# michaelwillett/GPU-ICP-SLAM

Hardware: AMD Instinct MI355X
Metric: particle-scan evals/sec (1081 beams x N particles), full particleFilter step, KD path (higher is better)
Workload: dtype f32; 1 GPU; synthetic 1081-beam scans, 100000 particles/GPU, 100000-point KD map, full SLAM step (disperse+score+weights+ICP/SVD+map update+resample); particles_global=100000, parallelism=particles sharded x1, map replicated, kd_size_end=191383

## Files before the change

gpu-icp-slam_amd/csrc/kd_cells.hip.inc:

```

#define PF_CELL_SUB 2
#define PF_CELL_WIN (2560 * PF_CELL_SUB)
#define PF_CELL_LIST_CAP (1 << 19)
#define PF_CELL_POOL_CAP (1 << 22)
#define PF_CELL_MAXC 12
#define PF_CELL_RUN 32
#define PF_CELL_MAXR 14
#define PF_CELL_MARK_MAX 4096
#define PF_CELL_PENDING 0xFFFFFFFFu
#define PF_CELL_FALLBACK 0xFFFFFFFEu
enum { PF_CS_COUNT = 0, PF_CS_POOL, PF_CS_SNAP, PF_CS_PAD3, PF_CS_LIST_CAP, PF_CS_POOL_CAP, PF_CS_FLAGS, PF_CS_PAD, PF_CS_ROWS, PF_CS_N1, PF_CS_N2,
       PF_CS_NONE, PF_CS_CUR_FRESH, PF_CS_CUR_EXT, PF_CS_CUR_REUSED, PF_CS_CUR_CLAIMED, PF_CS_WORDS = 32,
       PF_CS_OX = 128, PF_CS_OY = 129, PF_CS_ALLOC = 256 };
#define PF_CF_LIST_FULL 1
#define PF_CF_POOL_FULL 2
#define PF_CF_NEED_ORIGIN 4
#define PF_CF_FAR 8
#define PF_CELL_DRIFT_MAX 120
#define PF_REC_WORDS 96
#define PF_REC_TERM 4
#define PF_REC_CAND 20
#define PF_REC_PAR 36
#define PF_REC_RC 52
#define PF_REC_POOL 76
// ... 40 lines not shown
    const int k = S >> 1;
    cell_lo = (float)k * res;
    const float mid = cell_lo + 0.5f * res;
    lo = (S & 1) ? mid : cell_lo;
    hi = (S & 1) ? (float)(k + 1) * res : mid;
}
static_assert(PF_CELL_SUB == 2, "sub_index / sub_edges halve the lattice cell");

__device__ __forceinline__ bool beam_box(const pf::KdGroupBox &b, int j, float r, float &wxlo, float &wxhi, float &wylo, float &wyhi,
                                         const pf::AngleParts *T = nullptr, const pf::BeamParts *beams = nullptr)
{
    const float tc = 0.5f * (b.tlo + b.thi), dth = 0.5f * (b.thi - b.tlo);
    float cx, cy;
    if (T) beam_end_point(beams, j, r, tc, *T, cx, cy);
    else pf::clean_lidar_scan(j, r, tc, cx, cy);
    const float dd = dth + 1e-6f;
    const float eps = 2e-4f + 1e-5f * fabsf(r) + fabsf(r) * 2.0f * 1.1920929e-7f * (fabsf(tc) + 2.4f + dd);
    const float hx = (fabsf(cy) + fabsf(r) * dd) * dd + eps, hy = (fabsf(cx) + fabsf(r) * dd) * dd + eps;
    wxlo = b.xlo + cx - hx; wxhi = b.xhi + cx + hx; wylo = b.ylo + cy - hy; wyhi = b.yhi + cy + hy;
    return (wxlo == wxlo) && (wxhi == wxhi) && (wylo == wylo) && (wyhi == wyhi) && fabsf(wxlo) < 1e6f && fabsf(wxhi) < 1e6f &&
           fabsf(wylo) < 1e6f && fabsf(wyhi) < 1e6f && (wxhi - wxlo) < 4.0f && (wyhi - wylo) < 4.0f && fabsf(r) < PF_RANGE_NEVER;
}

#define PF_MARK_THREADS 256
#define PF_MARK_GROUPS 8
#define PF_MARK_CLAIMS 2048
#define PF_MARK_WORDS 4096
__global__ __launch_bounds__(PF_MARK_THREADS) void k_cells_mark(const pf::KdGroupBox *__restrict__ box, int groups,
                                                                const float *__restrict__ scan, int nb, CellGeom geo, unsigned *tab,
                                                                int *__restrict__ list, int *cs, const pf::AngleParts *__restrict__ gparts,
                                                                const pf::BeamParts *__restrict__ beams, unsigned long long *__restrict__ probe = nullptr)
{
    pf_stamp(probe);
    __shared__ unsigned bm[PF_MARK_WORDS];
    __shared__ int s_red[4][PF_MARK_THREADS / 64];
    const int t = threadIdx.x, lane = t & 63, wave = t >> 6, j = blockIdx.x;
    const int ox = cs[PF_CS_OX], oy = cs[PF_CS_OY];
    const float r = scan[j];
    int kx0[PF_MARK_GROUPS], kx1[PF_MARK_GROUPS], ky0[PF_MARK_GROUPS], ky1[PF_MARK_GROUPS];
    int ux0 = INT_MAX, ux1 = INT_MIN, uy0 = INT_MAX, uy1 = INT_MIN;
#pragma unroll
    for (int q = 0; q < PF_MARK_GROUPS; q++) {
        const int g = blockIdx.y * (PF_MARK_THREADS * PF_MARK_GROUPS) + q * PF_MARK_THREADS + t;
        kx0[q] = ky0[q] = INT_MAX;
        kx1[q] = ky1[q] = INT_MIN;
        if (g < groups) {
            float wxlo, wxhi, wylo, wyhi;
            const pf::AngleParts T = gparts[g];
            if (beam_box(box[g], j, r, wxlo, wxhi, wylo, wyhi, &T, beams)) {
                const int okx = ox >> 1, oky = oy >> 1, wk = PF_CELL_WIN / PF_CELL_SUB;
                const int a0 = max(lattice_floor(wxlo, geo.resx, geo.invx) - okx, 0), a1 = min(lattice_floor(wxhi, geo.resx, geo.invx) - okx, wk - 1);
                const int b0 = max(lattice_floor(wylo, geo.resy, geo.invy) - oky, 0), b1 = min(lattice_floor(wyhi, geo.resy, geo.invy) - oky, wk - 1);
                if (a0 <= a1 && b0 <= b1 && (long long)(a1 - a0 + 1) * (b1 - b0 + 1) <= PF_CELL_MARK_MAX) {
                    kx0[q] = a0; kx1[q] = a1; ky0[q] = b0; ky1[q] = b1;
// ... 4 lines not shown
    }
    for (int off = 32; off >= 1; off >>= 1) {
        ux0 = min(ux0, __shfl_xor(ux0, off, 64)); ux1 = max(ux1, __shfl_xor(ux1, off, 64));
        uy0 = min(uy0, __shfl_xor(uy0, off, 64)); uy1 = max(uy1, __shfl_xor(uy1, off, 64));
    }
    if (lane == 0) { s_red[0][wave] = ux0; s_red[1][wave] = ux1; s_red[2][wave] = uy0; s_red[3][wave] = uy1; }
    __syncthreads();
    for (int k = 0; k < PF_MARK_THREADS / 64; k++) {
        ux0 = min(ux0, s_red[0][k]); ux1 = max(ux1, s_red[1][k]); uy0 = min(uy0, s_red[2][k]); uy1 = max(uy1, s_red[3][k]);
    }
    if (ux0 > ux1) return;
    const int nx = ux1 - ux0 + 1;
    const long long bits = (long long)nx * (uy1 - uy0 + 1);
    __shared__ int s_claim[PF_MARK_CLAIMS];
    __shared__ int s_nclaim, s_base;
    if (t == 0) s_nclaim = 0;
    __syncthreads();
    auto claim = [&](int idx) {
        if (atomicCAS(&tab[idx], 0u, PF_CELL_PENDING) == 0u) {
            const int k = atomicAdd(&s_nclaim, 1);
            if (k < PF_MARK_CLAIMS) s_claim[k] = idx;
            else {
                const int pos = atomicAdd(&cs[PF_CS_COUNT], 1);
                if (pos < cs[PF_CS_LIST_CAP]) list[pos] = idx;
                else {
                    atomicExch(&tab[idx], PF_CELL_FALLBACK);
                    atomicOr(&cs[PF_CS_FLAGS], PF_CF_LIST_FULL);
                }
            }
        }
    };
    auto flush = [&]() {
        __syncthreads();
        const int nc = min(s_nclaim, PF_MARK_CLAIMS);
        if (t == 0 && nc > 0) {
            s_base = atomicAdd(&cs[PF_CS_COUNT], nc);
            atomicAdd(&cs[PF_CS_CUR_CLAIMED], nc);
        }
        __syncthreads();
        for (int k = t; k < nc; k += PF_MARK_THREADS) {
            const int pos = s_base + k;
            if (pos < cs[PF_CS_LIST_CAP]) list[pos] = s_claim[k];
            else {
                atomicExch(&tab[s_claim[k]], PF_CELL_FALLBACK);
                atomicOr(&cs[PF_CS_FLAGS], PF_CF_LIST_FULL);
            }
        }
    };
    if (bits > (long long)PF_MARK_WORDS * 32) {
#pragma unroll
        for (int q = 0; q < PF_MARK_GROUPS; q++) {
            if (kx0[q] > kx1[q] || (long long)(kx1[q] - kx0[q] + 1) * (ky1[q] - ky0[q] + 1) > PF_CELL_MARK_MAX) continue;
            for (int cy = ky0[q]; cy <= ky1[q]; cy++)
                for (int cx = kx0[q]; cx <= kx1[q]; cx++) claim(2 * cy * PF_CELL_WIN + 2 * cx);
        }
        flush();
        return;
    }
    const int words = (int)((bits + 31) >> 5);
    for (int w = t; w < words; w += PF_MARK_THREADS) bm[w] = 0u;
    __syncthreads();
#pragma unroll
    for (int q = 0; q < PF_MARK_GROUPS; q++)
        for (int cy = ky0[q]; cy <= ky1[q]; cy++) {
            const int b0 = (cy - uy0) * nx - ux0 + kx0[q], b1 = b0 + (kx1[q] - kx0[q]);
            for (int w = b0 >> 5; w <= (b1 >> 5); w++) {
// ... 624 lines not shown
#undef S_RY
__device__ __forceinline__ float cell_dist2(const uint4 cd, float wx, float wy)
{
    typedef float f32x2 __attribute__((ext_vector_type(2)));
    const f32x2 nxy = {__uint_as_float(cd.x), __uint_as_float(cd.y)};
    const f32x2 pxy = {wx, wy};
    const f32x2 d = nxy - pxy;
    const f32x2 dd = d * d;
    return dd.x + dd.y;
}
__device__ __forceinline__ bool cell_visit(const uint4 cd, float wx, float wy, float &sBest)
{
    const float s = cell_dist2(cd, wx, wy);
    const float sGuard = sBest * PF_GUARD_K;
    bool take = s < sGuard;
    const bool inBand = (s < sBest) != take;
    if (__builtin_amdgcn_ballot_w64(inBand) != 0ull) {
        float sb = sBest;
        asm volatile("" : "+v"(sb));
        take = take | (inBand && pf::fsqrt(s) < pf::fsqrt(sb));
    }
    sBest = take ? s : sBest;
    return take;
}

#define PF_ROW_SLACK 4
template <bool CENSUS = false, int GUARD = 1>
__global__ __launch_bounds__(64) void k_score_kd_cells(const float *__restrict__ px, const float *__restrict__ py,
                                                       const float *__restrict__ pth, int n, const float *__restrict__ scan,
                                                       const pf::BeamParts *__restrict__ beams, int nb, int beams_per_chunk, pf::KdView tree,
                                                       CellGeom geo, const unsigned *__restrict__ tab, const uint4 *__restrict__ pool,
                                                       const int *__restrict__ cs, const int *__restrict__ order, int direct,
                                                       float *__restrict__ out, int out_mode, pf::KdCensus *__restrict__ census = nullptr,
                                                       unsigned long long *__restrict__ probe = nullptr, const double2 *__restrict__ tparts = nullptr)
{
    pf_stamp(probe);
    const int g = blockIdx.x, slot = g * 64 + threadIdx.x;
    const int j0 = blockIdx.y * beams_per_chunk;
    const int j1 = min(nb, j0 + beams_per_chunk);
    const bool real = slot < n;
    const int i = order ? order[min(slot, n - 1)] : min(slot, n - 1);
    const float x = px[i], y = py[i], th = pth[i];
    pf::AngleParts T;
    if (tparts) {
        const double2 tp = tparts[i];
        T.c = tp.x;
// ... 144 lines not shown
```

gpu-icp-slam_amd/csrc/pfslam_frame.hip.inc:

```

#define PF_FRAME_RING 4
enum { PF_FS_BOUND = 0, PF_FS_WALKED = 4, PF_FS_TICKET = 8, PF_FS_ICP = 9, PF_FS_WORDS = 16 };
enum { PF_WC_WALLS = 0, PF_WC_NEW, PF_WC_FLAGS, PF_WC_SIZE, PF_WC_WORDS = 4 };

enum { PF_FL_REDUCED = 0, PF_FL_TREE, PF_FL_ORDER, PF_FL_ICP, PF_FL_SCAN, PF_FL_FTAIL, PF_FL_POSEG , PF_FL_WORDS = 8 };
__device__ __forceinline__ void flag_store(int *word, int ticket) { __hip_atomic_store(word, ticket, __ATOMIC_RELEASE, __HIP_MEMORY_SCOPE_AGENT); }
__device__ __forceinline__ bool flag_wait(const int *word, int ticket, int *err)
{
    const unsigned long long t0 = wall_clock64(), limit = g_gate_ticks;
    while (__hip_atomic_load(word, __ATOMIC_ACQUIRE, __HIP_MEMORY_SCOPE_AGENT) - ticket < 0) {
        __builtin_amdgcn_s_sleep(8);
        if (wall_clock64() - t0 > limit) {
            if (err) __hip_atomic_store(err, ticket, __ATOMIC_RELAXED, __HIP_MEMORY_SCOPE_SYSTEM);
            return false;
        }
    }
    return true;
}
__global__ void k_gate(const int *__restrict__ word, int ticket, int *__restrict__ err)
{
    if (threadIdx.x == 0) flag_wait(word, ticket, err);
}
__global__ void k_gate_signal(int *__restrict__ done_word, int done_ticket, const int *__restrict__ word, int ticket, int *__restrict__ err)
{
    if (threadIdx.x != 0) return;
    flag_store(done_word, done_ticket);
// ... 421 lines not shown
            wy = roundf(pf::fdiv(wy, resy));
            wx += (float)cx;
            wy += (float)cy;
            if (wx >= 0 && wx < dimx && wy >= 0 && wy < dimy) key = (uint32_t)(int)(wx * dimx + wy);
        }
    }
#pragma unroll
    for (int k = 2; k <= 64; k <<= 1)
#pragma unroll
        for (int q = k >> 1; q > 0; q >>= 1) {
            const uint32_t other = (uint32_t)__shfl_xor((int)key, q, 64);
            const bool asc = (lane & k) == 0, lower = (lane & q) == 0;
            key = (lower == asc) ? min(key, other) : max(key, other);
        }
    runs_g[j] = key;
    keys_s[j] = 0xFFFFFFFFu;
    if (probe && blockIdx.x == 0 && lane == 0) probe[PB_WALLS_KEYS - PB_WALLS] = wall_clock64();
}

template <bool PLANAR>
__global__ __launch_bounds__(64) void k_walls_rank_traverse(const uint32_t *__restrict__ runs_g, int sort_n, const float *__restrict__ pose, int dimx, float resx,
                                                            float resy, float scalex, float scaley, pf::KdView tree, uint32_t *__restrict__ keys_s,
                                                            float2 *__restrict__ xy_s, int *__restrict__ c2_s, int *__restrict__ leaf_s,
                                                            int *__restrict__ new_s, unsigned long long *__restrict__ probe, int split)
{
    pf_stamp(probe);
    extern __shared__ uint32_t s_dyn[];
    uint32_t *runs = s_dyn;
    const int lane = threadIdx.x, n_runs = sort_n >> 6, mine = blockIdx.x / split, per = 64 / split, pos = (blockIdx.x % split) * per + lane;
    for (int i = lane; i < sort_n; i += 64) runs[i] = runs_g[i];
    __syncthreads();
    if (lane >= per) return;
    const int i = mine * 64 + pos;
    const uint32_t key = runs[i];
    if (key == 0xFFFFFFFFu) return;
    int rank = pos;
    bool dup = pos > 0 && runs[i - 1] == key;
    for (int r0 = 0; r0 < n_runs; r0 += 4) {
        int lo[4] = {0, 0, 0, 0};
        uint32_t pk[4];
        bool on[4];
#pragma unroll
        for (int u = 0; u < 4; u++) {
            const int r = r0 + u;
            on[u] = r < n_runs && r != mine && !(r > mine && key == 0u);
            pk[u] = r < mine ? key : key - 1u;
        }
#pragma unroll
        for (int step = 32; step >= 1; step >>= 1)
#pragma unroll
            for (int u = 0; u < 4; u++)
                if (on[u]) lo[u] += (runs[(r0 + u) * 64 + lo[u] + step - 1] <= pk[u]) ? step : 0;
#pragma unroll
        for (int u = 0; u < 4; u++)
            if (on[u]) {
                const int cnt = lo[u] + ((lo[u] == 63 && runs[(r0 + u) * 64 + 63] <= pk[u]) ? 1 : 0);
                rank += cnt;
                if (r0 + u < mine && cnt > 0 && runs[(r0 + u) * 64 + cnt - 1] == key) dup = true;
            }
    }
    if (dup) return;
    const float4 p = cell_to_point((int)key, dimx, resx, resy, scalex, scaley, pose[0], pose[1]);
    int leaf;
    const int b = pf::kd_resume<PLANAR, false, true>(tree, p.x, p.y, p.z, INFINITY, 0, 0, nullptr, &leaf);
    const float cellDiag = pf::fsqrt(resx * resx + resy * resy), minDist = cellDiag / 2.0f;
    keys_s[rank] = key;
    xy_s[rank] = make_float2(p.x, p.y);
    c2_s[rank] = b;
    leaf_s[rank] = leaf;
    new_s[rank] = node_dist(tree, b, p) > minDist ? 1 : 0;
}

template <bool PLANAR>
__global__ __launch_bounds__(256) void k_free_traverse(float4 *__restrict__ free_pts, int *__restrict__ free_idx, int free_cap, int wall_cap,
                                                       const int *__restrict__ counts, pf::KdView tree, int zero_tail, float *kw, float resx,
                                                       float resy, const int *__restrict__ bound_ptr, unsigned long long *__restrict__ probe)
{
    pf_stamp(probe);
    const int n_wall = min(counts[0], wall_cap), n_free = min(counts[1], free_cap);
    const int bound = *bound_ptr;
    const float cellDiag = pf::fsqrt(resx * resx + resy * resy);
    for (int i = blockIdx.x * 256 + threadIdx.x; i < n_free; i += gridDim.x * 256) {
        float4 p = free_pts[i];
        if (zero_tail && i >= n_wall) {
            p = make_float4(0.0f, 0.0f, 0.0f, 0.0f);
            free_pts[i] = p;
        }
// ... 517 lines not shown
                     c.multi ? (const long long *)h->gkeys : (const long long *)nullptr, c.multi ? (const float *)h->gpose : (const float *)nullptr, h->world, h->stride};
    return c;
}
#define FV_EDGE_WAIT(st, word, ev, back)                                                                                                      \
    do {                                                                                                                                      \
        if (c.gates) {                                                                                                                        \
            hipLaunchKernelGGL(k_gate, dim3(1), dim3(64), 0, st, (const int *)(c.fl + (word)), seq - (back), h->gate_err_dev);                \
            HIPCHK(hipGetLastError());                                                                                                        \
        } else HIPCHK(hipStreamWaitEvent(st, ev, 0));                                                                                         \
    } while (0)

static int fv_cells_passes(pfslam_handle *h, const FvCtx &c)
{
    const int seq = c.seq, s4 = c.s4, groups = c.groups;
    hipStream_t K = c.K;
    const bool mark_early = h->mark_early != 0;
    if (!c.sync_cells) {
        if (mark_early) FV_EDGE_WAIT(K, PF_FL_ORDER, h->ev_order, 0);
        else FV_EDGE_WAIT(K, PF_FL_REDUCED, h->ev_reduced, 0);
    }
    hipLaunchKernelGGL(k_group_box, dim3(groups), dim3(64), 0, K, h->x_frame, h->y_frame, h->th_frame, h->n, (const int *)c.order, h->group_box, h->group_parts, h->d_sigma);
    const int per_block = PF_MARK_THREADS * PF_MARK_GROUPS;
    hipLaunchKernelGGL(k_cells_mark, dim3(h->nb, (groups + per_block - 1) / per_block), dim3(PF_MARK_THREADS), 0, K, (const pf::KdGroupBox *)h->group_box,
                       groups, (const float *)h->scan, h->nb, c.geo, h->cell_tab, h->cell_list, h->cell_state, (const pf::AngleParts *)h->group_parts,
                       (const pf::BeamParts *)h->beam_angle, PB(PB_MARK));
    HIPCHK(hipGetLastError());
    HIPCHK(hipEventRecord(h->ev_marked_r[s4], K));
    if (!c.sync_cells && h->pipe_live) FV_EDGE_WAIT(K, PF_FL_TREE, h->ev_tree2, 1);
    if (c.sync_cells) {
        h->cells_passes++;
        hipLaunchKernelGGL(k_cells_update<true>, dim3(PF_CELLS_GRID), dim3(64), 0, K, c.tv, c.geo, h->cell_tab, (const int *)h->cell_list, h->cell_state, h->cell_pool,
                           h->cell_rec, h->cells_gen, (const int *)nullptr, 0, 0, 0, CellPass{nullptr, nullptr, nullptr, nullptr, 0}, PB(PB_WALK));
        hipLaunchKernelGGL(k_fs_walked, dim3(1), dim3(64), 0, K, h->fs, (const int *)h->cell_state);
    } else {
        hipLaunchKernelGGL(k_cells_update<false>, dim3(PF_CELLS_WALK_GRID), dim3(64), 0, K, c.tv, c.geo, h->cell_tab, (const int *)h->cell_list, h->cell_state,
                           h->cell_pool, h->cell_rec, h->cells_gen, (const int *)nullptr, 0, 0, 0,
                           CellPass{h->fs + PF_FS_WALKED + ((seq - 1) & 3), h->fs + PF_FS_WALKED + s4, nullptr, h->fs + PF_FS_BOUND + s4, 0}, PB(PB_WALK));
    }
    HIPCHK(hipGetLastError());
    HIPCHK(hipEventRecord(h->ev_walked_r[s4], K));
    return 0;
}

static int frame_v2_begin(pfslam_handle *h, int frame, const float *scan_host, int used, int bpc, bool sharded)
{
    CHK(frame_alloc(h));
    if (!h->cell_tab) CHK(cells_alloc(h));
// ... 170 lines not shown
        if (!sync_cells && h->mark_early == 0) CHK(fv_cells_passes(h, c));
        const int sort_n = (h->nb + 63) / 64 * 64;
        const size_t lds = (size_t)sort_n * 9 * sizeof(uint32_t);
        if (!h->walls_attr_set) {
            HIPCHK(hipFuncSetAttribute((const void *)k_walls<0>, hipFuncAttributeMaxDynamicSharedMemorySize, (int)lds));
            HIPCHK(hipFuncSetAttribute((const void *)k_walls<3>, hipFuncAttributeMaxDynamicSharedMemorySize, (int)lds));
            h->walls_attr_set = true;
        }
        const int cx = (int)roundf(0.5f * h->dimx + h->cfg.map_res_x / 2), cy = (int)roundf(0.5f * h->dimy + h->cfg.map_res_y / 2);
        const int wait_poseg = c.multi ? 1 : 0;
#define PF_WALLS_ARGS dim3(1), dim3(1024), lds, C, (const float *)h->scan, (const pf::BeamParts *)h->beam_angle, h->nb, sort_n, c.psrc, h->start, h->pose, c.stats_next, \
                      cx, cy, h->dimx, h->dimy, h->cfg.map_res_x, h->cfg.map_res_y, h->cfg.map_scale_x, h->cfg.map_scale_y, c.tv, h->hot, h->parent, h->kz, h->kw,   \
                      h->kd_state, h->kd_cap, sort_n, h->wall_c2, h->wcounts, h->fs + PF_FS_BOUND + ((seq + 1) & 3), (const int *)h->cell_state, h->cell_touched
        if (h->planar == 0) {
            hipLaunchKernelGGL(k_walls<0>, PF_WALLS_ARGS, PB(PB_WALLS), h->wall_xy2, h->wall_leaf2, h->wall_new2, gates ? fl : (int *)nullptr, seq, h->gate_err_dev,
                               (const uint32_t *)nullptr, (const int *)nullptr, wait_poseg, h->trig);
        } else {
            hipLaunchKernelGGL(k_wall_runs, dim3(sort_n / 64), dim3(64), 0, C, (const float *)h->scan, (const pf::BeamParts *)h->beam_angle, h->nb, c.psrc, h->start, h->pose,
                               c.stats_next, cx, cy, h->dimx, h->dimy, h->cfg.map_res_x, h->cfg.map_res_y, h->wall_runs, h->wall_keys_s, PB(PB_WALLS),
                               gates ? fl : (int *)nullptr, seq, h->gate_err_dev, wait_poseg, h->trig);
            const int walls_split = 4;
            hipLaunchKernelGGL(k_walls_rank_traverse<true>, dim3(sort_n / 64 * walls_split), dim3(64), (size_t)sort_n * 4, C, (const uint32_t *)h->wall_runs, sort_n,
                               (const float *)h->pose, h->dimx, h->cfg.map_res_x, h->cfg.map_res_y, h->cfg.map_scale_x, h->cfg.map_scale_y, c.tv, h->wall_keys_s,
                               h->wall_xy2, h->wall_c2s, h->wall_leaf2, h->wall_new2, PB(PB_WALLS_REP), walls_split);
            hipLaunchKernelGGL(k_walls<3>, PF_WALLS_ARGS, PB(PB_WALLS), h->wall_xy2, h->wall_leaf2, h->wall_new2, (int *)nullptr, seq, (int *)nullptr,
                               (const uint32_t *)h->wall_keys_s, (const int *)h->wall_c2s);
        }
#undef PF_WALLS_ARGS
        HIPCHK(hipGetLastError());
        if (!gates) HIPCHK(hipEventRecord(h->ev_tree2, C));
        const int recut = h->cells_passes > 0 && h->cells_passes % PF_CELLS_RECUT_EVERY == 0 ? 1 : 0;
        if (recut) HIPCHK(hipMemsetAsync(h->cell_state + PF_CS_POOL, 0, 4, C));
        hipLaunchKernelGGL(k_cells_update<true>, dim3(PF_CELLS_GRID), dim3(64), 0, C, c.tv, c.geo, h->cell_tab, (const int *)h->cell_list, h->cell_state, h->cell_pool,
                           h->cell_rec, h->cells_gen, (const int *)h->cell_touched, (int)(h->cells_passes & 15), recut, 0,
                           CellPass{nullptr, nullptr, h->fs + PF_FS_WALKED + ((seq - (sync_cells ? 0 : lag)) & 3), nullptr, h->fault}, PB(PB_UPDATE),
                           gates ? fl + PF_FL_TREE : (int *)nullptr, seq);
        HIPCHK(hipGetLastError());
        h->cells_passes++;
    }
    {
        FV_EDGE_WAIT(P, PF_FL_REDUCED, h->ev_reduced, 0);
        if (!serial) {
            HIPCHK(hipStreamWaitEvent(P, h->ev_marked_r[(seq - 1) & 3], 0));
            HIPCHK(hipStreamWaitEvent(P, h->ev_walked_r[(seq + 1 - lag) & 3], 0));
        }
        if (c.sharded) {
            hipLaunchKernelGGL(k_weights_apply_sharded, dim3((h->n + 255) / 256), dim3(256), 0, P, h->w, h->wm, (const float *)h->fit, h->n, h->goff, mirror_count(h),
// ... 107 lines not shown
```

gpu-icp-slam_amd/csrc/pfslam_hip.hip:

```cpp
#include "../../include/pfslam.h"
#include "kd_device.h"
#include "pf_math.h"

#include <hip/hip_runtime.h>

#include <algorithm>
#include <atomic>
#include <deque>
#include <thread>
#include <cmath>
#include <cstdio>
#include <chrono>
#include <cstring>
#include <string>
#include <vector>

#define PF_LIDAR_RANGE 20.0f
#define PF_RANGE_NEVER 28.4f
#define PF_FREE_WEIGHT (-1)
#define PF_OCCUPIED_WEIGHT 4
#define PF_EFFECTIVE_PARTICLES .7
#define PF_CLAMP_VAL 113.0f
#define PF_SUM_EXACT 16777216.0f
#define PF_SVD_EPSILON 0.00001f
// ... 156 lines not shown
    bool icp_forked = false;
    bool icp_delta_ready = false;
    bool masks_cleared = false;
    bool stats_clean = false;
    int timing = 0;
    struct TimedSpan { hipEvent_t a, b; int slot; bool keep_b = false; };
    std::vector<hipEvent_t> ev_pool;
    std::vector<TimedSpan> ev_pending;
    hipEvent_t phase_ev = nullptr;
    double timer_ms[PF_TIMER_SLOTS] = {0};
    long timer_count[PF_TIMER_SLOTS] = {0};
    pf::KdCensus *d_census = nullptr;
    pf::KdCensus *census_store = nullptr, *census_log = nullptr;
    int census_n = 0;
    pf::KdPlanRow *plan = nullptr;
    size_t plan_rows = 0;
    bool plan_valid = false;
    pf::KdGroupBox *group_box = nullptr;
    pf::AngleParts *group_parts = nullptr;
    bool lattice_ok = false;
    bool cells_valid = false;
    unsigned *cell_tab = nullptr;
    int *cell_list = nullptr, *cell_state = nullptr, *cell_rec = nullptr;
    int *cell_touched = nullptr;
    uint4 *cell_pool = nullptr;
    bool cells_wipe_pending = false;
    float cloud_sigma = 0.0f;
    float *d_sigma = nullptr;
    float theta_bound = 0.0f, theta_shift = 0.0f;
    int theta_shift_seq = 0;
    bool cells_suspended = false;
    int cells_full_frame = -1;
    bool balance_external = false;
    int cells_wipe_seq = 0;
    bool score_on_aux = false;
    bool scored_on_aux = false;
    hipEvent_t ev_scored = nullptr;
    bool cells_async = false;
    long cells_wipes = 0;
    long cells_passes = 0;
    int cells_gen = 0;
    hipEvent_t ev_boxes = nullptr;
    hipEvent_t ev_marked = nullptr;
    bool mark_on_aux = false;
    hipStream_t istream = nullptr;
    hipEvent_t ev_tree = nullptr;
// ... 30 lines not shown
    hipEvent_t ev_marked_r[4] = {nullptr, nullptr, nullptr, nullptr}, ev_walked_r[4] = {nullptr, nullptr, nullptr, nullptr};
    hipEvent_t ev_tail[3] = {nullptr, nullptr, nullptr};
    int fault = 0;
    int stable_order = 0;
    int *order_tmp = nullptr;
    int mark_early = 1;
    int gates = 1;
    bool ftail_recorded = false;
    int *flags = nullptr;
    int *gate_err = nullptr, *gate_err_dev = nullptr;
    const float *x_frame = nullptr, *y_frame = nullptr, *th_frame = nullptr;
    bool shift_pending = false;
    bool balance_done = false;
    bool walls_attr_set = false;
    unsigned long long *probe = nullptr;
    int probe_frames = 0;
};
#define PF_PROBE_SLOTS 32
enum { PB_ICP = 0, PB_MOTION, PB_SCATTER, PB_BOX, PB_MARK, PB_WALK, PB_SCORE, PB_REDUCE, PB_WALLS, PB_UPDATE, PB_WEIGHTS, PB_APPLY, PB_GATHER, PB_RAYS, PB_COUNT,
       PB_LISTS, PB_FREE, PB_WALLW, PB_REDUCE_LAST, PB_WALLS_KEYS, PB_WALLS_SORTED, PB_WALLS_TRAV, PB_WALLS_END, PB_WALLS_REP, PB_ICP_SOLVE, PB_ICP_END, PB_UPDATE_END, PB_REDUCE_END, PB_END };
static const char *const pb_names[PB_END] = {"K icp", "P motion+cells", "P scatter", "K boxes", "K mark", "K walk", "C scan-match", "C reduce", "C walls+insert",
                                             "C cells update", "P weights", "P scan apply", "P sample+gather", "F rays", "F count", "F lists", "F free pass", "F wall weights",
                                             "C reduce: last wg", "C walls: keys", "C walls: sorted", "C walls: traversed", "C walls: end", "C walls: traversal launch", "K icp: solve", "K icp: end", "C cells update: last wg ends", "C reduce: last wg ends"};
static_assert(PB_END <= PF_PROBE_SLOTS, "probe slots");


__global__ __launch_bounds__(256) void k_motion(float *__restrict__ x, float *__restrict__ y,
                                                float *__restrict__ th, float *__restrict__ w,
                                                const float *__restrict__ wm, int n, int frame, int goff, int trig = 0)
{
    int i = blockIdx.x * 256 + threadIdx.x;
    if (i >= n) return;
    w[i] = wm[i];
    uint32_t e2 = pf::engine_seed(frame, goff + i, 0);
    const float sx = 0.015, sy = 0.015, st = .01;
    float nx = pf::normal(e2, 0.0f, sx, trig != 0);
    float ny = pf::normal(e2, 0.0f, sy, trig != 0);
    float nt = pf::normal(e2, 0.0f, st, trig != 0);
    x[i] += nx;
    y[i] += ny;
    th[i] += nt;
}

__global__ void k_beam_angles(pf::BeamParts *__restrict__ beams, int nb)
{
    const int j = blockIdx.x * blockDim.x + threadIdx.x;
    if (j >= nb) return;
// ... 624 lines not shown
    if (h->cstream) { (void)hipStreamSynchronize(h->cstream); (void)hipStreamDestroy(h->cstream); }
    if (h->istream) { (void)hipStreamSynchronize(h->istream); (void)hipStreamDestroy(h->istream); }
    if (h->ev_tree) (void)hipEventDestroy(h->ev_tree);
    if (h->ev_scored) (void)hipEventDestroy(h->ev_scored);
    if (h->ev_walked) (void)hipEventDestroy(h->ev_walked);
    if (h->topo_stream) { (void)hipStreamSynchronize(h->topo_stream); (void)hipStreamDestroy(h->topo_stream); }
    if (h->ev_fork) (void)hipEventDestroy(h->ev_fork);
    if (h->ev_join) (void)hipEventDestroy(h->ev_join);
    if (h->ev_mapfork) (void)hipEventDestroy(h->ev_mapfork);
    if (h->ev_map) (void)hipEventDestroy(h->ev_map);
    for (auto &e : h->ev_pool) (void)hipEventDestroy(e);
    for (auto &e : h->ev_pending) { (void)hipEventDestroy(e.a); if (!e.keep_b) (void)hipEventDestroy(e.b); }
    if (h->phase_ev) (void)hipEventDestroy(h->phase_ev);
    if (h->d_census) (void)hipFree(h->d_census);
    if (h->census_store) (void)hipFree(h->census_store);
    if (h->plan) (void)hipFree(h->plan);
    if (h->group_box) (void)hipFree(h->group_box);
    if (h->group_parts) (void)hipFree(h->group_parts);
    if (h->cell_tab) (void)hipFree(h->cell_tab);
    if (h->cell_list) (void)hipFree(h->cell_list);
    if (h->cell_state) (void)hipFree(h->cell_state);
    if (h->cell_pool) (void)hipFree(h->cell_pool);
    if (h->cell_rec) (void)hipFree(h->cell_rec);
    if (h->cell_touched) (void)hipFree(h->cell_touched);
    if (h->ev_boxes) (void)hipEventDestroy(h->ev_boxes);
    if (h->ev_marked) (void)hipEventDestroy(h->ev_marked);
    if (h->beam_angle) (void)hipFree(h->beam_angle);
    frame_free(h);
    if (h->own_stream && h->stream) (void)hipStreamDestroy(h->stream);
    delete h;
    g_live_handles.fetch_sub(1);
    return 0;
}

extern "C" int pfslam_set_stream(pfslam_handle *h, void *hip_stream)
{
    if (!h) return fail("null handle");
    CHK(settle(h));
    if (h->stream) HIPCHK(hipStreamSynchronize(h->stream));
    if (h->own_stream && h->stream) {
        HIPCHK(hipStreamSynchronize(h->stream));
        HIPCHK(hipStreamDestroy(h->stream));
    }
    h->stream = (hipStream_t)hip_stream;
    h->own_stream = false;
    h->gates_tested = false;
// ... 499 lines not shown
    const float Dside = h->n <= 400000 ? 64.0f : 128.0f;
    const float box_cells = 2.0f * (6.4f * h->cloud_sigma / Dside) * cbrtf(64.0f * Dside * Dside * Dside / (float)h->n) / std::min(h->cfg.map_res_x, h->cfg.map_res_y);
    const bool narrow = h->variant == 3 || !(box_cells > PF_CELLS_BOX_MAX);
    const bool use_cells = organised && h->lattice_ok && h->variant != 4 && !h->cells_suspended && narrow;
    if (use_plan) *use_plan = !use_cells && h->planar && h->variant != 2 && (h->n >= plan_min_n || h->variant >= 3);
    return use_cells;
}
__global__ void k_reduce_partials_minmax(const float *partial, int n, int chunks, const int *order, float *fit, int goff, long long *stats,
                                         const float *x, const float *y, const float *th, int p16);
__global__ void k_reduce_partials_minmax_wide(const float *partial, int n, int chunks, const int *order, float *fit, long long *stats);
template <typename T> __global__ void k_minmax(const T *fit, int n, int goff, long long *stats);
static int join_icp(pfslam_handle *h);
static int launch_stats_reset(pfslam_handle *h, hipStream_t st);

static int cells_alloc(pfslam_handle *h)
{
    CHK(dalloc(&h->cell_tab, (size_t)PF_CELL_WIN * PF_CELL_WIN));
    CHK(dalloc(&h->cell_list, (size_t)PF_CELL_LIST_CAP));
    HIPCHK(hipMemsetAsync(h->cell_list, 0, (size_t)PF_CELL_LIST_CAP * 4, h->stream));
    CHK(dalloc(&h->cell_state, PF_CS_ALLOC));
    HIPCHK(hipMemsetAsync(h->cell_state, 0, PF_CS_ALLOC * 4, h->stream));
    CHK(dalloc(&h->cell_rec, (size_t)PF_CELL_LIST_CAP * PF_REC_WORDS));
    HIPCHK(hipMemsetAsync(h->cell_rec, 0, (size_t)PF_CELL_LIST_CAP * PF_REC_WORDS * 4, h->stream));
    CHK(dalloc(&h->cell_pool, (size_t)PF_CELL_POOL_CAP + PF_ROW_SLACK));
    CHK(dalloc(&h->cell_touched, (size_t)h->max_wall + 1));
    HIPCHK(hipMemsetAsync(h->cell_touched, 0, 4, h->stream));
    HIPCHK(pf_event_create(&h->ev_boxes, hipEventDisableTiming));
    HIPCHK(pf_event_create(&h->ev_marked, hipEventDisableTiming));
    HIPCHK(pf_event_create(&h->ev_walked, hipEventDisableTiming));
    h->cells_wipe_pending = true;
    return 0;
}

static int launch_score(pfslam_handle *h, bool fuse_minmax = false, pf::KdCensus *census = nullptr, bool sharded = false)
{
    if (h->kd_size <= 0) return fail("pfslam_score_kd: no map loaded");
    const int chunks = score_chunks(h);
    const int bpc = (h->nb + chunks - 1) / chunks;
    const int used = (h->nb + bpc - 1) / bpc;
    float *out = h->fit;
    if (used > 1) {
        const size_t need = (size_t)used * h->n;
        if (need > h->partial_elems) {
            if (h->partial) HIPCHK(hipFree(h->partial));
            h->partial = nullptr;
            CHK(dalloc(&h->partial, need));
// ... 44 lines not shown
        }
        hipLaunchKernelGGL(k_group_box, dim3(groups), dim3(64), 0, h->stream, h->x, h->y, h->th, h->n, order, h->group_box, h->group_parts, h->d_sigma);
    }
    hipEvent_t t_a = nullptr, t_b = nullptr;
    if (h->timing && !census) {
        CHK(timer_event(h, &t_a));
        CHK(timer_event(h, &t_b));
        HIPCHK(hipEventRecord(t_a, h->stream));
    }
    const CellArgs ca{h->cell_tab, h->cell_list, h->cell_state, h->cell_pool, h->cell_rec};
    if (use_cells) {
        hipStream_t st = h->stream;
        if (!cells_sync) {
            HIPCHK(hipEventRecord(h->ev_boxes, h->stream));
            HIPCHK(hipStreamWaitEvent(h->cstream, h->ev_boxes, 0));
            st = h->cstream;
        }
        if (h->update_unsnapped) {
            HIPCHK(hipStreamWaitEvent(st, h->ev_map, 0));
            h->update_unsnapped = false;
        }
        const int groups = (h->n + 63) / 64, per_block = PF_MARK_THREADS * PF_MARK_GROUPS;
        hipLaunchKernelGGL(k_cells_mark, dim3(h->nb, (groups + per_block - 1) / per_block), dim3(PF_MARK_THREADS), 0, st,
                           (const pf::KdGroupBox *)h->group_box, groups, (const float *)h->scan, h->nb, geo, h->cell_tab, h->cell_list, h->cell_state,
                           (const pf::AngleParts *)h->group_parts, (const pf::BeamParts *)h->beam_angle);
        if (!cells_sync) {
            HIPCHK(hipEventRecord(h->ev_marked, st));
            h->mark_on_aux = true;
            HIPCHK(hipStreamWaitEvent(st, h->ev_map, 0));
            hipLaunchKernelGGL(k_cells_update<false>, dim3(PF_CELLS_WALK_GRID), dim3(64), 0, st, kd_view(h), geo, ca.tab, (const int *)ca.list, ca.cs, ca.pool, ca.rec, h->cells_gen, (const int *)nullptr, 0);
            HIPCHK(hipEventRecord(h->ev_walked, st));
            h->walk_pending = true;
            h->cells_snap = true;
        }
        HIPCHK(hipGetLastError());
    }
    const bool on_aux = h->score_on_aux && use_cells && !cells_sync && fuse_minmax && !census && !sharded;
    h->scored_on_aux = on_aux;
    struct StreamSwap {
        pfslam_handle *h;
        hipStream_t keep;
        ~StreamSwap() { h->stream = keep; }
    } swap_guard{h, h->stream};
    if (on_aux) {
        HIPCHK(hipStreamWaitEvent(h->aux, h->ev_boxes, 0));
        h->stream = h->aux;
    }
// ... 473 lines not shown
    HIPCHK(hipSetDevice(h->cfg.device));
    CHK(settle(h));
    float *d_xyz = nullptr;
    int *d_best = nullptr;
    CHK(dalloc(&d_xyz, (size_t)n * 3));
    CHK(dalloc(&d_best, (size_t)n));
    HIPCHK(hipMemcpyAsync(d_xyz, xyz_host, (size_t)n * 12, hipMemcpyHostToDevice, h->stream));
    bool planar = h->planar;
    if (planar)
        for (int i = 0; i < n; i++)
            if (xyz_host[3 * i + 2] != 0.0f) { planar = false; break; }
    if (planar)
        hipLaunchKernelGGL(k_traverse<true>, dim3((n + 255) / 256), dim3(256), 0, h->stream, d_xyz, n, kd_view(h), d_best);
    else
        hipLaunchKernelGGL(k_traverse<false>, dim3((n + 255) / 256), dim3(256), 0, h->stream, d_xyz, n, kd_view(h), d_best);
    HIPCHK(hipGetLastError());
    HIPCHK(hipMemcpyAsync(best_host, d_best, (size_t)n * 4, hipMemcpyDeviceToHost, h->stream));
    HIPCHK(hipStreamSynchronize(h->stream));
    HIPCHK(hipFree(d_xyz));
    HIPCHK(hipFree(d_best));
    return 0;
}

extern "C" int pfslam_debug_math(pfslam_handle *h, int which, const float *in_host, int n, float *out_host)
{
    if (!h || !in_host || !out_host || n <= 0) return fail("pfslam_debug_math: bad argument");
    HIPCHK(hipSetDevice(h->cfg.device));
    CHK(settle(h));
    const int per = which == 0 || which == 6 || which == 7 ? 2 : 1;
    float *d_in = nullptr, *d_out = nullptr;
    CHK(dalloc(&d_in, (size_t)n));
    CHK(dalloc(&d_out, (size_t)n * per));
    HIPCHK(hipMemcpyAsync(d_in, in_host, (size_t)n * 4, hipMemcpyHostToDevice, h->stream));
    hipLaunchKernelGGL(k_debug_math, dim3((n + 255) / 256), dim3(256), 0, h->stream, which, d_in, n, d_out);
    HIPCHK(hipGetLastError());
    HIPCHK(hipMemcpyAsync(out_host, d_out, (size_t)n * per * 4, hipMemcpyDeviceToHost, h->stream));
    HIPCHK(hipStreamSynchronize(h->stream));
    HIPCHK(hipFree(d_in));
    HIPCHK(hipFree(d_out));
    return 0;
}

extern "C" int pfslam_device_ptr(pfslam_handle *h, int which, void **ptr, size_t *bytes)
{
    if (!h || !ptr || !bytes) return fail("pfslam_device_ptr: bad argument");
    const size_t n = h->n;
    switch (which) {
    case 0: *ptr = h->stats; *bytes = 64; break;
    case 1: *ptr = h->fit; *bytes = n * 4; break;
    case 2: *ptr = h->x; *bytes = n * 4; break;
    case 3: *ptr = h->y; *bytes = n * 4; break;
// ... 39 lines not shown
```

Before: 173.1 million particle-scan evals/s.

## Reuse per-cell candidate records to shortcut KD traversal for wall points

Adds a lattice-to-record index (rec_of) filled by the cell mark kernel, so wall-point insertion can look up the already-computed cell candidate record and resolve its nearest neighbour directly. A full kd_resume traversal runs only when the record gives no exact hit. This is meant to cut KD traversal cost in the walls rank/traverse kernel. In exchange it adds a global scatter in the mark kernel, a 16 MB index buffer, per-wave stat atomics, and a debug checker kernel.

```diff
diff --git a/gpu-icp-slam_amd/csrc/kd_cells.hip.inc b/gpu-icp-slam_amd/csrc/kd_cells.hip.inc
--- a/gpu-icp-slam_amd/csrc/kd_cells.hip.inc
+++ b/gpu-icp-slam_amd/csrc/kd_cells.hip.inc
@@ -86,14 +86,22 @@
            fabsf(wylo) < 1e6f && fabsf(wyhi) < 1e6f && (wxhi - wxlo) < 4.0f && (wyhi - wylo) < 4.0f && fabsf(r) < PF_RANGE_NEVER;
 }
 
+#define PF_CELL_LAT (PF_CELL_WIN / PF_CELL_SUB)
+__device__ __forceinline__ int cell_lat_index(int tab_idx)
+{
+    const int cyw = tab_idx / PF_CELL_WIN, cxw = tab_idx - cyw * PF_CELL_WIN;
+    return (cyw / PF_CELL_SUB) * PF_CELL_LAT + cxw / PF_CELL_SUB;
+}
+
 #define PF_MARK_THREADS 256
 #define PF_MARK_GROUPS 8
 #define PF_MARK_CLAIMS 2048
 #define PF_MARK_WORDS 4096
 __global__ __launch_bounds__(PF_MARK_THREADS) void k_cells_mark(const pf::KdGroupBox *__restrict__ box, int groups,
                                                                 const float *__restrict__ scan, int nb, CellGeom geo, unsigned *tab,
-                                                                int *__restrict__ list, int *cs, const pf::AngleParts *__restrict__ gparts,
-                                                                const pf::BeamParts *__restrict__ beams, unsigned long long *__restrict__ probe = nullptr)
+                                                                int *__restrict__ list, int *__restrict__ rec_of, int *cs,
+                                                                const pf::AngleParts *__restrict__ gparts, const pf::BeamParts *__restrict__ beams,
+                                                                unsigned long long *__restrict__ probe = nullptr)
 {
     pf_stamp(probe);
     __shared__ unsigned bm[PF_MARK_WORDS];
@@ -144,8 +152,10 @@
             if (k < PF_MARK_CLAIMS) s_claim[k] = idx;
             else {
                 const int pos = atomicAdd(&cs[PF_CS_COUNT], 1);
-                if (pos < cs[PF_CS_LIST_CAP]) list[pos] = idx;
-                else {
+                if (pos < cs[PF_CS_LIST_CAP]) {
+                    list[pos] = idx;
+                    rec_of[cell_lat_index(idx)] = pos;
+                } else {
                     atomicExch(&tab[idx], PF_CELL_FALLBACK);
                     atomicOr(&cs[PF_CS_FLAGS], PF_CF_LIST_FULL);
                 }
@@ -162,8 +172,10 @@
         __syncthreads();
         for (int k = t; k < nc; k += PF_MARK_THREADS) {
             const int pos = s_base + k;
-            if (pos < cs[PF_CS_LIST_CAP]) list[pos] = s_claim[k];
-            else {
+            if (pos < cs[PF_CS_LIST_CAP]) {
+                list[pos] = s_claim[k];
+                rec_of[cell_lat_index(s_claim[k])] = pos;
+            } else {
                 atomicExch(&tab[s_claim[k]], PF_CELL_FALLBACK);
                 atomicOr(&cs[PF_CS_FLAGS], PF_CF_LIST_FULL);
             }
@@ -834,6 +846,47 @@
     }
     sBest = take ? s : sBest;
     return take;
+}
+
+enum { PF_WR_HIT = 0, PF_WR_OPEN, PF_WR_UNPUBLISHED, PF_WR_DEAD, PF_WR_KINDS };
+struct WallRecords { const int *cs, *rec_of, *list, *rec_base; int gen; int *stats; unsigned long long *probe; };
+template <bool ANY_BEST = false>
+__device__ __forceinline__ int cell_record_descent(const pf::KdView &tree, const WallRecords &wr, float resx, float resy, float qx, float qy,
+                                                   int &best, int &leaf, float *s_out = nullptr)
+{
+    const int Kx = (int)rintf(pf::fdiv(qx, resx)), Ky = (int)rintf(pf::fdiv(qy, resy));
+    if (!(abs(Kx) < PF_LATTICE_KMAX && abs(Ky) < PF_LATTICE_KMAX && (float)Kx * resx == qx && (float)Ky * resy == qy)) return PF_WR_UNPUBLISHED;
+    const int cxw = PF_CELL_SUB * Kx - wr.cs[PF_CS_OX], cyw = PF_CELL_SUB * Ky - wr.cs[PF_CS_OY];
+    if ((unsigned)cxw >= (unsigned)PF_CELL_WIN || (unsigned)cyw >= (unsigned)PF_CELL_WIN) return PF_WR_UNPUBLISHED;
+    const int cell = cyw * PF_CELL_WIN + cxw;
+    const int r = wr.rec_of[cell_lat_index(cell)];
+    if ((unsigned)r >= (unsigned)PF_CELL_LIST_CAP) return PF_WR_UNPUBLISHED;
+    const int *rec = wr.rec_base + (size_t)r * PF_REC_WORDS;
+    const int owner = wr.list[r];
+    const int4 hd = *(const int4 *)rec;
+    int4 cv[PF_CELL_MAXU / 4];
+#pragma unroll
+    for (int q = 0; q < PF_CELL_MAXU / 4; q++) cv[q] = *(const int4 *)(rec + PF_REC_CAND + 4 * q);
+    const int m = hd.z & 0xff, fl = hd.z >> 16;
+    if (owner != cell || hd.w != wr.gen || (fl & PF_RF_FRESH)) return PF_WR_UNPUBLISHED;
+    if ((fl & PF_RF_DEAD) || m < 1 || m > PF_CELL_MAXU) return PF_WR_DEAD;
+    const int ci[PF_CELL_MAXU] = {cv[0].x, cv[0].y, cv[0].z, cv[0].w, cv[1].x, cv[1].y, cv[1].z, cv[1].w,
+                                  cv[2].x, cv[2].y, cv[2].z, cv[2].w, cv[3].x, cv[3].y, cv[3].z, cv[3].w};
+    uint4 nd[PF_CELL_MAXU];
+#pragma unroll
+    for (int k = 0; k < PF_CELL_MAXU; k++)
+        if (k < m) nd[k] = tree.hot[ci[k]];
+    float sBest = cell_dist2(nd[0], qx, qy);
+    int b = ci[0];
+#pragma unroll
+    for (int k = 1; k < PF_CELL_MAXU; k++)
+        if (k < m && cell_visit(nd[k], qx, qy, sBest)) b = ci[k];
+    if (s_out) *s_out = sBest;
+    if (ANY_BEST || sBest == 0.0f) {
+        best = b;
+        leaf = hd.y;
+    }
+    return sBest == 0.0f ? PF_WR_HIT : PF_WR_OPEN;
 }
 
 #define PF_ROW_SLACK 4
diff --git a/gpu-icp-slam_amd/csrc/pfslam_frame.hip.inc b/gpu-icp-slam_amd/csrc/pfslam_frame.hip.inc
--- a/gpu-icp-slam_amd/csrc/pfslam_frame.hip.inc
+++ b/gpu-icp-slam_amd/csrc/pfslam_frame.hip.inc
@@ -1,7 +1,8 @@
 
 #define PF_FRAME_RING 4
 enum { PF_FS_BOUND = 0, PF_FS_WALKED = 4, PF_FS_TICKET = 8, PF_FS_ICP = 9, PF_FS_WORDS = 16 };
-enum { PF_WC_WALLS = 0, PF_WC_NEW, PF_WC_FLAGS, PF_WC_SIZE, PF_WC_WORDS = 4 };
+enum { PF_WC_WALLS = 0, PF_WC_NEW, PF_WC_FLAGS, PF_WC_SIZE, PF_WC_WORDS = 8 };
+static_assert(PF_WC_REC == PF_WC_SIZE + 1 && PF_WC_REC + PF_WR_KINDS <= PF_WC_WORDS, "wall counters");
 
 enum { PF_FL_REDUCED = 0, PF_FL_TREE, PF_FL_ORDER, PF_FL_ICP, PF_FL_SCAN, PF_FL_FTAIL, PF_FL_POSEG , PF_FL_WORDS = 8 };
 __device__ __forceinline__ void flag_store(int *word, int ticket) { __hip_atomic_store(word, ticket, __ATOMIC_RELEASE, __HIP_MEMORY_SCOPE_AGENT); }
@@ -469,7 +470,8 @@
 __global__ __launch_bounds__(64) void k_walls_rank_traverse(const uint32_t *__restrict__ runs_g, int sort_n, const float *__restrict__ pose, int dimx, float resx,
                                                             float resy, float scalex, float scaley, pf::KdView tree, uint32_t *__restrict__ keys_s,
                                                             float2 *__restrict__ xy_s, int *__restrict__ c2_s, int *__restrict__ leaf_s,
-                                                            int *__restrict__ new_s, unsigned long long *__restrict__ probe, int split)
+                                                            int *__restrict__ new_s, unsigned long long *__restrict__ probe, int split,
+                                                            WallRecords wr = WallRecords{nullptr, nullptr, nullptr, nullptr, 0, nullptr, nullptr})
 {
     pf_stamp(probe);
     extern __shared__ uint32_t s_dyn[];
@@ -508,8 +510,18 @@
     }
     if (dup) return;
     const float4 p = cell_to_point((int)key, dimx, resx, resy, scalex, scaley, pose[0], pose[1]);
-    int leaf;
-    const int b = pf::kd_resume<PLANAR, false, true>(tree, p.x, p.y, p.z, INFINITY, 0, 0, nullptr, &leaf);
+    int leaf = -1, b = -1, kind = PF_WR_KINDS;
+    if (PLANAR && wr.rec_of) {
+        kind = cell_record_descent(tree, wr, resx, resy, p.x, p.y, b, leaf);
+        for (int k = 0; k < PF_WR_KINDS; k++) {
+            const unsigned long long mk = __ballot(kind == k);
+            if (mk != 0ull && kind == k && lane == __ffsll((long long)mk) - 1) {
+                atomicAdd(&wr.stats[k], __popcll(mk));
+                if (wr.probe) atomicAdd(&wr.probe[k], (unsigned long long)__popcll(mk));
+            }
+        }
+    }
+    if (kind != PF_WR_HIT) b = pf::kd_resume<PLANAR, false, true>(tree, p.x, p.y, p.z, INFINITY, 0, 0, nullptr, &leaf);
     const float cellDiag = pf::fsqrt(resx * resx + resy * resy), minDist = cellDiag / 2.0f;
     keys_s[rank] = key;
     xy_s[rank] = make_float2(p.x, p.y);
@@ -1073,7 +1085,7 @@
     hipLaunchKernelGGL(k_group_box, dim3(groups), dim3(64), 0, K, h->x_frame, h->y_frame, h->th_frame, h->n, (const int *)c.order, h->group_box, h->group_parts, h->d_sigma);
     const int per_block = PF_MARK_THREADS * PF_MARK_GROUPS;
     hipLaunchKernelGGL(k_cells_mark, dim3(h->nb, (groups + per_block - 1) / per_block), dim3(PF_MARK_THREADS), 0, K, (const pf::KdGroupBox *)h->group_box,
-                       groups, (const float *)h->scan, h->nb, c.geo, h->cell_tab, h->cell_list, h->cell_state, (const pf::AngleParts *)h->group_parts,
+                       groups, (const float *)h->scan, h->nb, c.geo, h->cell_tab, h->cell_list, h->cell_rec_of, h->cell_state, (const pf::AngleParts *)h->group_parts,
                        (const pf::BeamParts *)h->beam_angle, PB(PB_MARK));
     HIPCHK(hipGetLastError());
     HIPCHK(hipEventRecord(h->ev_marked_r[s4], K));
@@ -1290,7 +1302,11 @@
             const int walls_split = 4;
             hipLaunchKernelGGL(k_walls_rank_traverse<true>, dim3(sort_n / 64 * walls_split), dim3(64), (size_t)sort_n * 4, C, (const uint32_t *)h->wall_runs, sort_n,
                                (const float *)h->pose, h->dimx, h->cfg.map_res_x, h->cfg.map_res_y, h->cfg.map_scale_x, h->cfg.map_scale_y, c.tv, h->wall_keys_s,
-                               h->wall_xy2, h->wall_c2s, h->wall_leaf2, h->wall_new2, PB(PB_WALLS_REP), walls_split);
+                               h->wall_xy2, h->wall_c2s, h->wall_leaf2, h->wall_new2, PB(PB_WALLS_REP), walls_split,
+                               (h->wall_records && h->fault == 0)
+                                   ? WallRecords{(const int *)h->cell_state, (const int *)h->cell_rec_of, (const int *)h->cell_list, (const int *)h->cell_rec, h->cells_gen,
+                                                 h->wcounts + PF_WC_REC, PB(PB_REC_KINDS)}
+                                   : WallRecords{nullptr, nullptr, nullptr, nullptr, 0, nullptr, nullptr});
             hipLaunchKernelGGL(k_walls<3>, PF_WALLS_ARGS, PB(PB_WALLS), h->wall_xy2, h->wall_leaf2, h->wall_new2, (int *)nullptr, seq, (int *)nullptr,
                                (const uint32_t *)h->wall_keys_s, (const int *)h->wall_c2s);
         }
diff --git a/gpu-icp-slam_amd/csrc/pfslam_hip.hip b/gpu-icp-slam_amd/csrc/pfslam_hip.hip
--- a/gpu-icp-slam_amd/csrc/pfslam_hip.hip
+++ b/gpu-icp-slam_amd/csrc/pfslam_hip.hip
@@ -202,6 +202,8 @@
     bool cells_valid = false;
     unsigned *cell_tab = nullptr;
     int *cell_list = nullptr, *cell_state = nullptr, *cell_rec = nullptr;
+    int *cell_rec_of = nullptr;
+    int wall_records = 1;
     int *cell_touched = nullptr;
     uint4 *cell_pool = nullptr;
     bool cells_wipe_pending = false;
@@ -278,7 +280,9 @@
 static const char *const pb_names[PB_END] = {"K icp", "P motion+cells", "P scatter", "K boxes", "K mark", "K walk", "C scan-match", "C reduce", "C walls+insert",
                                              "C cells update", "P weights", "P scan apply", "P sample+gather", "F rays", "F count", "F lists", "F free pass", "F wall weights",
                                              "C reduce: last wg", "C walls: keys", "C walls: sorted", "C walls: traversed", "C walls: end", "C walls: traversal launch", "K icp: solve", "K icp: end", "C cells update: last wg ends", "C reduce: last wg ends"};
-static_assert(PB_END <= PF_PROBE_SLOTS, "probe slots");
+#define PB_REC_KINDS PB_END
+static_assert(PB_END + 4 <= PF_PROBE_SLOTS, "probe slots");
+#define PF_WC_REC 4
 
 
 __global__ __launch_bounds__(256) void k_motion(float *__restrict__ x, float *__restrict__ y,
@@ -949,6 +953,7 @@
     if (h->cell_state) (void)hipFree(h->cell_state);
     if (h->cell_pool) (void)hipFree(h->cell_pool);
     if (h->cell_rec) (void)hipFree(h->cell_rec);
+    if (h->cell_rec_of) (void)hipFree(h->cell_rec_of);
     if (h->cell_touched) (void)hipFree(h->cell_touched);
     if (h->ev_boxes) (void)hipEventDestroy(h->ev_boxes);
     if (h->ev_marked) (void)hipEventDestroy(h->ev_marked);
@@ -1494,6 +1499,8 @@
     HIPCHK(hipMemsetAsync(h->cell_state, 0, PF_CS_ALLOC * 4, h->stream));
     CHK(dalloc(&h->cell_rec, (size_t)PF_CELL_LIST_CAP * PF_REC_WORDS));
     HIPCHK(hipMemsetAsync(h->cell_rec, 0, (size_t)PF_CELL_LIST_CAP * PF_REC_WORDS * 4, h->stream));
+    CHK(dalloc(&h->cell_rec_of, (size_t)PF_CELL_LAT * PF_CELL_LAT));
+    HIPCHK(hipMemsetAsync(h->cell_rec_of, 0xff, (size_t)PF_CELL_LAT * PF_CELL_LAT * 4, h->stream));
     CHK(dalloc(&h->cell_pool, (size_t)PF_CELL_POOL_CAP + PF_ROW_SLACK));
     CHK(dalloc(&h->cell_touched, (size_t)h->max_wall + 1));
     HIPCHK(hipMemsetAsync(h->cell_touched, 0, 4, h->stream));
@@ -1584,7 +1591,7 @@
         }
         const int groups = (h->n + 63) / 64, per_block = PF_MARK_THREADS * PF_MARK_GROUPS;
         hipLaunchKernelGGL(k_cells_mark, dim3(h->nb, (groups + per_block - 1) / per_block), dim3(PF_MARK_THREADS), 0, st,
-                           (const pf::KdGroupBox *)h->group_box, groups, (const float *)h->scan, h->nb, geo, h->cell_tab, h->cell_list, h->cell_state,
+                           (const pf::KdGroupBox *)h->group_box, groups, (const float *)h->scan, h->nb, geo, h->cell_tab, h->cell_list, h->cell_rec_of, h->cell_state,
                            (const pf::AngleParts *)h->group_parts, (const pf::BeamParts *)h->beam_angle);
         if (!cells_sync) {
             HIPCHK(hipEventRecord(h->ev_marked, st));
@@ -2104,11 +2111,109 @@
     return 0;
 }
 
+__global__ __launch_bounds__(64) void k_wall_records_check(pf::KdView tree, WallRecords wr, float resx, float resy, unsigned long long *__restrict__ out)
+{
+    const int count = min(wr.cs[PF_CS_COUNT], wr.cs[PF_CS_LIST_CAP]);
+    const int ox = wr.cs[PF_CS_OX], oy = wr.cs[PF_CS_OY];
+    unsigned long long c[8] = {0};
+    for (int r = blockIdx.x * 64 + threadIdx.x; r < count; r += gridDim.x * 64) {
+        const int cell = wr.list[r];
+        const int cyw = cell / PF_CELL_WIN, cxw = cell - cyw * PF_CELL_WIN;
+        const int Kx = (ox + cxw) >> 1, Ky = (oy + cyw) >> 1;
+        const float qx = (float)Kx * resx, qy = (float)Ky * resy;
+        c[0]++;
+        int fbest = 0, fleaf = -1;
+        {
+            float sBest = INFINITY;
+            for (int head = 0; head >= 0;) {
+                const uint4 nd = tree.hot[head];
+                if (cell_visit(nd, qx, qy, sBest)) fbest = head;
+                const uint32_t axis = nd.z >> 30;
+                const bool lt = axis == 0 ? qx < __uint_as_float(nd.x) : (axis == 1 ? qy < __uint_as_float(nd.y) : false);
+                fleaf = head * 2 + (lt ? 0 : 1);
+                head = lt ? pf::hot_left(nd.z) : (int)nd.w;
+            }
+        }
+        int wleaf = -1;
+        const int wb = pf::kd_resume<true, false, true>(tree, qx, qy, 0.0f, INFINITY, 0, 0, nullptr, &wleaf);
+        int b = -1, leaf = -1;
+        const int kind = cell_record_descent<true>(tree, wr, resx, resy, qx, qy, b, leaf);
+        if (kind == PF_WR_HIT) {
+            c[1]++;
+            if (b != wb || leaf != wleaf) c[2]++;
+        } else if (kind == PF_WR_OPEN) {
+            c[3]++;
+            if (b != fbest) c[4]++;
+        } else c[kind == PF_WR_DEAD ? 6 : 5]++;
+        if ((kind == PF_WR_HIT || kind == PF_WR_OPEN) && (leaf != wleaf || wleaf != fleaf)) c[7]++;
+    }
+    for (int k = 0; k < 8; k++) {
+        unsigned long long v = c[k];
+        for (int off = 32; off >= 1; off >>= 1) v += __shfl_xor(v, off, 64);
+        if ((threadIdx.x & 63) == 0 && v) atomicAdd(&out[k], v);
+    }
+}
+static int debug_wall_records(pfslam_handle *h, int which, const float *in_host, int n, float *out_host)
+{
+    int *out = (int *)out_host;
+    for (int k = 0; k < n; k++) out[k] = 0;
+    if (which == 100) {
+        out[0] = h->wall_records;
+        h->wall_records = in_host[0] != 0.0f ? 1 : 0;
+        return 0;
+    }
+    if (which == 102) {
+        if (!h->wcounts) return 0;
+        int v[PF_WR_KINDS];
+        HIPCHK(hipMemcpyAsync(v, h->wcounts + PF_WC_REC, sizeof(v), hipMemcpyDeviceToHost, h->stream));
+        HIPCHK(hipStreamSynchronize(h->stream));
+        for (int k = 0; k < PF_WR_KINDS && k < n; k++) out[k] = v[k];
+        return 0;
+    }
+    if (which == 103) {
+        if (!h->wcounts || !h->wall_keys_s || !h->planar) return 0;
+        const int sort_n = (h->nb + 63) / 64 * 64;
+        int nw = 0;
+        HIPCHK(hipMemcpyAsync(&nw, h->wcounts, 4, hipMemcpyDeviceToHost, h->stream));
+        HIPCHK(hipStreamSynchronize(h->stream));
+        if (nw < 0 || nw > sort_n || n < 2 + nw + 3 * sort_n) return fail("pfslam_debug_math 103: room for 2 + walls + 3 x places words");
+        std::vector<int> key(sort_n), leaf(sort_n), isnew(sort_n);
+        HIPCHK(hipMemcpy(out + 2, h->wall_c2, (size_t)nw * 4, hipMemcpyDeviceToHost));
+        HIPCHK(hipMemcpy(key.data(), h->wall_keys_s, (size_t)sort_n * 4, hipMemcpyDeviceToHost));
+        HIPCHK(hipMemcpy(leaf.data(), h->wall_leaf2, (size_t)sort_n * 4, hipMemcpyDeviceToHost));
+        HIPCHK(hipMemcpy(isnew.data(), h->wall_new2, (size_t)sort_n * 4, hipMemcpyDeviceToHost));
+        out[0] = nw;
+        out[1] = sort_n;
+        for (int i = 0; i < sort_n; i++) {
+            const bool on = key[i] != -1;
+            out[2 + nw + 3 * i] = key[i];
+            out[2 + nw + 3 * i + 1] = on ? leaf[i] : 0;
+            out[2 + nw + 3 * i + 2] = on ? isnew[i] : 0;
+        }
+        return 0;
+    }
+    if (!h->cell_tab || !h->cells_valid || h->cells_wipe_pending || !h->planar || h->kd_size <= 0) return 0;
+    unsigned long long *d = nullptr;
+    CHK(dalloc(&d, 8));
+    HIPCHK(hipMemsetAsync(d, 0, 64, h->stream));
+    hipLaunchKernelGGL(k_wall_records_check, dim3(512), dim3(64), 0, h->stream, kd_view(h),
+                       WallRecords{(const int *)h->cell_state, (const int *)h->cell_rec_of, (const int *)h->cell_list, (const int *)h->cell_rec, h->cells_gen, nullptr, nullptr},
+                       h->cfg.map_res_x, h->cfg.map_res_y, d);
+    HIPCHK(hipGetLastError());
+    unsigned long long v[8];
+    HIPCHK(hipMemcpyAsync(v, d, 64, hipMemcpyDeviceToHost, h->stream));
+    HIPCHK(hipStreamSynchronize(h->stream));
+    HIPCHK(hipFree(d));
+    for (int k = 0; k < 8 && k < n; k++) out[k] = (int)v[k];
+    return 0;
+}
+
 extern "C" int pfslam_debug_math(pfslam_handle *h, int which, const float *in_host, int n, float *out_host)
 {
     if (!h || !in_host || !out_host || n <= 0) return fail("pfslam_debug_math: bad argument");
     HIPCHK(hipSetDevice(h->cfg.device));
     CHK(settle(h));
+    if (which >= 100 && which <= 103) return debug_wall_records(h, which, in_host, n, out_host);
     const int per = which == 0 || which == 6 || which == 7 ? 2 : 1;
     float *d_in = nullptr, *d_out = nullptr;
     CHK(dalloc(&d_in, (size_t)n));
```

Result: no change. 172.2 million particle-scan evals/s (-0.5%).
